# meuleman/epilogos

Hardware: NVIDIA B200
Metric: bins/sec for expected+scores (S2) (higher is better)
Workload: dtype int64+f64

## Files before the change

### epilogos_b200/csrc/common.cuh

```cuda
#pragma once
#include <cuda_runtime.h>
#include <cuda.h>
#include <stddef.h>
#include <stdint.h>
#include <stdio.h>
#include <string.h>

#include "../../include/epilogos_b200.h"

namespace epi {

void set_error(const char* fmt, ...);
int check_device();

#define EPI_CUDA(call)                                                                        \
    do {                                                                                      \
        cudaError_t e__ = (call);                                                             \
        if (e__ != cudaSuccess) {                                                             \
            epi::set_error("%s failed at %s:%d: %s", #call, __FILE__, __LINE__,               \
                           cudaGetErrorString(e__));                                          \
            return 1;                                                                         \
        }                                                                                     \
    } while (0)

#define EPI_REQUIRE(cond, ...)                                                                \
    do {                                                                                      \
        if (!(cond)) {                                                                        \
            epi::set_error(__VA_ARGS__);                                                      \
            return 2;                                                                         \
        }                                                                                     \
    } while (0)

int sm_count();
int persistent_grid(int64_t ntiles, int per_sm);

constexpr int S1_TABLE_MAX_WIDTH = 4095;

struct PrepFlags {
    int has_zero;
};

struct K5TcConsts {
    double dg[EPI_MAX_STATES];
    double scale;
    double cst;
    int has_zero;
    uint32_t m1, m8, m16;
    int fbits;
};

struct DeviceWorkspace {
    unsigned long long reduce_slots[64];
    double log2e[EPI_MAX_STATES * EPI_MAX_STATES];
    PrepFlags prep_flags;
    int s3_symmetric;
    alignas(16) uint8_t k5tc_b_image[8 * EPI_MAX_STATES * 128];
    K5TcConsts k5tc_consts;
    alignas(8) double s1_v64[EPI_MAX_STATES * (S1_TABLE_MAX_WIDTH + 1)];
    alignas(8) float s1_v32[EPI_MAX_STATES * (S1_TABLE_MAX_WIDTH + 1)];
    alignas(8) float perm_v32[2][EPI_MAX_STATES * (S1_TABLE_MAX_WIDTH + 1)];
};
static_assert(offsetof(DeviceWorkspace, k5tc_b_image) % 16 == 0, "the B operand image is a bulk-copy source");
static_assert(offsetof(DeviceWorkspace, s1_v64) % 8 == 0 && offsetof(DeviceWorkspace, s1_v32) % 8 == 0,
              "the S1 value tables need 8-byte alignment");

DeviceWorkspace* device_workspace();

typedef CUresult (*tensor_map_encode_fn)(CUtensorMap*, CUtensorMapDataType, cuuint32_t, void*, const cuuint64_t*,
                                         const cuuint64_t*, const cuuint32_t*, const cuuint32_t*,
                                         CUtensorMapInterleave, CUtensorMapSwizzle, CUtensorMapL2promotion,
                                         CUtensorMapFloatOOBfill);
tensor_map_encode_fn get_tensor_map_encode();

int s1_value_table(const float* e, int K, int width, float* v32, double* v64, cudaStream_t st);

int launch_k2_tc(const uint16_t* cnt, int64_t bins, int K, int64_t* n1, int64_t* n2, cudaStream_t st);
int scores_s2_tc(const uint16_t* cnt, int64_t bins, int K, int width, int64_t perms, const float* e, int* zero_flag,
                 float* o32, double* o64, cudaStream_t st);
bool scores_s2_tc_eligible(int width);
int scores_s2_tc_fixed_point(const float* e, int K, int64_t perms, unsigned long long* mfix_dev, int* fbits_host,
                             cudaStream_t st);

#ifdef __CUDACC__

__device__ __forceinline__ uint32_t smem_u32(const void* p) {
    return static_cast<uint32_t>(__cvta_generic_to_shared(p));
}

__device__ __forceinline__ void mbar_init(uint64_t* bar, uint32_t count) {
    asm volatile("mbarrier.init.shared::cta.b64 [%0], %1;" ::"r"(smem_u32(bar)), "r"(count));
}
__device__ __forceinline__ void mbar_fence_init() {
    asm volatile("fence.mbarrier_init.release.cluster;" ::: "memory");
}
__device__ __forceinline__ void mbar_expect_tx(uint64_t* bar, uint32_t bytes) {
    asm volatile("mbarrier.arrive.expect_tx.shared::cta.b64 _, [%0], %1;" ::"r"(smem_u32(bar)), "r"(bytes)
                 : "memory");
}
__device__ __forceinline__ void mbar_arrive(uint64_t* bar) {
    asm volatile("mbarrier.arrive.shared::cta.b64 _, [%0];" ::"r"(smem_u32(bar)) : "memory");
}
// ... 84 lines not shown
```

### epilogos_b200/csrc/count_tile.cuh

```cuda
#pragma once
#include "tc05.cuh"

namespace epi {

#ifdef __CUDACC__

constexpr int T2_OP_BYTES = 128 * 128;
constexpr int T2_DRAIN = 256;

__device__ __forceinline__ uint64_t make_mnmajor_sw128_desc(uint32_t smem_addr) {
    uint64_t d = 0;
    d |= (uint64_t)((smem_addr >> 4) & 0x3fff);
    d |= (uint64_t)((128u >> 4) & 0x3fff) << 16;
    d |= (uint64_t)((1024u >> 4) & 0x3fff) << 32;
    d |= (uint64_t)1 << 46;
    d |= (uint64_t)2 << 61;
    return d;
}
constexpr uint32_t UMMA_A_MN_MAJOR = 1u << 15, UMMA_B_MN_MAJOR = 1u << 16;

template <int KT>
__device__ __forceinline__ void store_operand_row(uint8_t* row_ptr, int r, const uint32_t (&cw)[KT / 2], int ones_word,
                                                  uint32_t ones_val) {
    constexpr int NW = ((KT / 2 + 1 + 3) / 4) * 4;
// ... 25 lines not shown
        for (int i = 0; i < NW; ++i) t[i] = w[i];
#pragma unroll
        for (int i = 0; i < KT / 2; ++i) {
            if (i < NW - 1) cw[i] = __funnelshift_r(t[i], t[i + 1], sh);
            else if (i == NW - 1) cw[i] = (sh ? (t[i] >> 16) : t[i]) & 0xffffu;
            else cw[i] = 0u;
        }
    } else {
#pragma unroll
        for (int i = 0; i < KT / 2; ++i)
            cw[i] = (2 * i < K ? (uint32_t)row[2 * i] : 0u) | ((2 * i + 1 < K ? (uint32_t)row[2 * i + 1] : 0u) << 16);
    }
}
template <int KT>
__device__ __forceinline__ void load_count_row_guarded(const uint16_t* row, int K, bool live, uint32_t (&cw)[KT / 2]) {
#pragma unroll
    for (int i = 0; i < KT / 2; ++i)
        cw[i] = (live && 2 * i < K ? (uint32_t)row[2 * i] : 0u) | ((live && 2 * i + 1 < K ? (uint32_t)row[2 * i + 1] : 0u) << 16);
}

template <int NCOL>
__device__ __forceinline__ void drain_gram(uint32_t tmem_lane_base, int warp, int lane, int K, unsigned long long* n1,
                                           unsigned long long* n2) {
    uint32_t v[NCOL];
#pragma unroll
    for (int c0 = 0; c0 < NCOL; c0 += 16) {
        uint32_t t16[16];
        tmem_ld_32x16(tmem_lane_base + (uint32_t)c0, t16);
#pragma unroll
        for (int j = 0; j < 16; ++j) v[c0 + j] = t16[j];
    }
    const int m = warp * 32 + lane;
    const int s = m >> 1;
    const bool owner = (m & 1) == 0 && s < K;
    long long diag = 0, cnt1 = 0;
#pragma unroll
    for (int q = 0; q < NCOL / 2; ++q) {
        const uint32_t p0 = __shfl_down_sync(0xffffffffu, v[2 * q], 1), p1 = __shfl_down_sync(0xffffffffu, v[2 * q + 1], 1);
        const long long val = (long long)v[2 * q] + 256ll * (long long)v[2 * q + 1] + 256ll * ((long long)p0 + 256ll * (long long)p1);
        if (q == K) cnt1 = val;
        else if (q == s) diag = val;
        else if (owner && q < K && n2 != nullptr && val != 0) atomicAdd(&n2[s * K + q], (unsigned long long)val);
    }
    if (owner) {
        diag -= cnt1;
        if (n2 != nullptr && diag != 0) atomicAdd(&n2[s * K + s], (unsigned long long)diag);
        if (n1 != nullptr && cnt1 != 0) atomicAdd(&n1[s], (unsigned long long)cnt1);
    }
}


#endif

}
```

### epilogos_b200/csrc/scores.cu

```cuda
#include "common.cuh"

namespace epi {

constexpr int K5_THREADS = 256;
constexpr int K5_WARPS = K5_THREADS / 32;
constexpr int KT_MAX = EPI_MAX_STATES;

__constant__ __align__(16) double c_log2e[KT_MAX * KT_MAX];

__global__ void k5_prepare_kernel(const float* __restrict__ e, int rows, int cols, int kt, double* __restrict__ out,
                                  PrepFlags* flags) {
    __shared__ int zero;
    if (threadIdx.x == 0) zero = 0;
    __syncthreads();
    for (int i = threadIdx.x; i < rows * kt; i += blockDim.x) {
        const int s = i / kt, q = i - s * kt;
        double v = 0.0;
        if (q < cols) {
            const double ev = (double)e[s * cols + q];
            if (ev > 0.0) v = log2(ev);
            else zero = 1;
        }
        out[i] = v;
    }
    __syncthreads();
    if (threadIdx.x == 0) flags->has_zero = zero;
}

__device__ __forceinline__ double kl_direct(double obs, double e) {
    if (e == 0.0 || obs == 0.0) return 0.0;
    return obs * log2(obs / e);
}

struct WarpCountStream {
    const uint16_t* cnt;
    uint16_t* slab[2];
    uint64_t* bar;
    long long bins, ngroups, stride;
    int K, lane, buf;
    uint32_t phase[2];

    __device__ __forceinline__ void issue(long long g, int b) const {
        if (lane == 0 && g < ngroups && bins - g * 32 >= 32) {
            mbar_expect_tx(&bar[b], 64 * K);
            bulk_load_1d(slab[b], cnt + g * 32 * K, 64 * K, &bar[b]);
        }
    }
    __device__ __forceinline__ const uint16_t* acquire(long long g, int nvalid) {
        const int b = buf;
        buf ^= 1;
        issue(g + stride, b ^ 1);
        if (nvalid == 32) {
            mbar_wait(&bar[b], phase[b]);
            phase[b] ^= 1;
// ... 76 lines not shown
        if (out32 != nullptr) warp_store_scores(myf, out32 + bin0 * K, nvalid, K, lane);
        else __syncwarp();
    }
}

__global__ void __launch_bounds__(K5_THREADS) k5_s1_direct_kernel(const uint16_t* __restrict__ cnt, long long bins, int K,
                                                                  int width, const float* __restrict__ exp1,
                                                                  float* __restrict__ out32, double* __restrict__ out64) {
    const double dw = (double)width;
    const long long n = bins * K;
    for (long long i = blockIdx.x * (long long)blockDim.x + threadIdx.x; i < n; i += (long long)gridDim.x * blockDim.x) {
        const int s = (int)(i % K);
        const double v = kl_direct((double)cnt[i] / dw, (double)__ldg(exp1 + s));
        if (out32 != nullptr) out32[i] = (float)v;
        if (out64 != nullptr) out64[i] = v;
    }
}

template <int KT>
__global__ void __launch_bounds__(K5_THREADS) k5_s2_kernel(const uint16_t* __restrict__ cnt, long long bins, int K,
                                                           int width, double perms, const float* __restrict__ exp2,
                                                           const PrepFlags* __restrict__ flags, int force_direct,
                                                           float* __restrict__ out32, double* __restrict__ out64) {
    if (force_direct == 2 && !flags->has_zero) return;
    extern __shared__ __align__(128) uint8_t smem_raw[];
    uint16_t* cslab = reinterpret_cast<uint16_t*>(smem_raw);
    float* fslab = reinterpret_cast<float*>(smem_raw + K5_WARPS * 32 * K * 4);
    uint64_t* bars = reinterpret_cast<uint64_t*>(smem_raw + K5_WARPS * 32 * K * 8);

    const int tid = threadIdx.x, warp = tid >> 5, lane = tid & 31;
    if (tid == 0) {
        for (int i = 0; i < K5_WARPS * 2; ++i) mbar_init(&bars[i], 1);
        mbar_fence_init();
    }
    __syncthreads();
    const double lp = log2(perms);
    const double inv_perms = 1.0 / perms;
    const bool direct = force_direct || flags->has_zero;
    float* myf = fslab + warp * 32 * K;

    const long long ngroups = (bins + 31) / 32;
    WarpCountStream in{cnt, {cslab + warp * 64 * K, cslab + warp * 64 * K + 32 * K}, bars + warp * 2, bins, ngroups,
                       (long long)gridDim.x * K5_WARPS, K, lane, 0, {0u, 0u}};
    in.issue((long long)blockIdx.x * K5_WARPS + warp, 0);
    for (long long g = (long long)blockIdx.x * K5_WARPS + warp; g < ngroups; g += in.stride) {
        const long long bin0 = g * 32;
        const int nvalid = (int)((bins - bin0) < 32 ? (bins - bin0) : 32);
        const uint16_t* myc = in.acquire(g, nvalid);
        if (lane < nvalid) {
            const uint16_t* row = myc + lane * K;
            float* orow = myf + lane * K;
            if (direct) {
                for (int q = 0; q < K; ++q) {
                    const long long cq = row[q];
                    double sum = 0.0;
                    if (cq != 0) {
                        for (int s = 0; s < K; ++s) {
                            const long long cs = row[s];
                            const long long prod = (s == q) ? cs * (cs - 1) : cs * cq;
                            if (prod != 0) sum += kl_direct((double)prod / perms, (double)__ldg(exp2 + s * K + q));
                        }
                    }
                    orow[q] = (float)sum;
                    if (out64 != nullptr) out64[(bin0 + lane) * K + q] = sum;
                }
            } else {
                double cd[KT], mc[KT];
                double a = 0.0, w = 0.0;
#pragma unroll
                for (int s = 0; s < KT; ++s) {
                    const int c = s < K ? row[s] : 0;
                    cd[s] = (double)c;
                    const double l = c > 0 ? log2((double)c) : 0.0;
                    a = fma(cd[s], l, a);
                    w += cd[s];
                    mc[s] = 0.0;
                }
                const double2* le2 = reinterpret_cast<const double2*>(c_log2e);
#pragma unroll
                for (int s = 0; s < KT; ++s) {
#pragma unroll
                    for (int q = 0; q < KT; q += 2) {
                        const double2 m = le2[(s * KT + q) >> 1];
                        mc[q] = fma(cd[s], m.x, mc[q]);
                        mc[q + 1] = fma(cd[s], m.y, mc[q + 1]);
                    }
                }
                const double wm1 = w - 1.0;
// ... 75 lines not shown
    }
    EPI_CUDA(cudaGetLastError());
    return 0;
}

template <int KT>
static int launch_s2(const uint16_t* cnt, int64_t bins, int K, int width, int64_t perms, const float* e,
                     const PrepFlags* flags, int direct, float* o32, double* o64, cudaStream_t st) {
    auto kern = k5_s2_kernel<KT>;
    const size_t smem = (size_t)K5_WARPS * 32 * K * 8 + K5_WARPS * 16;
    EPI_CUDA(cudaFuncSetAttribute(kern, cudaFuncAttributeMaxDynamicSharedMemorySize, (int)smem));
    const int64_t ntiles = (bins + K5_THREADS - 1) / K5_THREADS;
    kern<<<persistent_grid(ntiles, 3), K5_THREADS, smem, st>>>(cnt, bins, K, width, (double)perms, e, flags, direct, o32,
                                                                o64);
    EPI_CUDA(cudaGetLastError());
    return 0;
}

template <int KT>
static int dispatch_s2(const uint16_t* cnt, int64_t bins, int K, int width, int64_t perms, const float* e, float* o32,
                       double* o64, int mode, cudaStream_t st) {
    const PrepFlags* flags = nullptr;
    if (mode == EPI_SCORE_TABLE && scores_s2_tc_eligible(width)) {
        DeviceWorkspace* ws = device_workspace();
        EPI_REQUIRE(ws != nullptr, "could not allocate the per-device workspace");
        PrepFlags* fl = &ws->prep_flags;
        if (int rc = scores_s2_tc(cnt, bins, K, width, perms, e, &fl->has_zero, o32, o64, st)) return rc;
        return launch_s2<KT>(cnt, bins, K, width, perms, e, fl, 2, o32, o64, st);
    }
    if (int rc = prepare_tables(e, K, K, KT, st, &flags)) return rc;
    return launch_s2<KT>(cnt, bins, K, width, perms, e, flags, mode == EPI_SCORE_DIRECT, o32, o64, st);
}

}

using namespace epi;

static int check_score_args(const void* cnt, int64_t bins, int K, int width, const void* e, int mode) {
    if (check_device()) return 3;
    EPI_REQUIRE(bins >= 0 && bins < (1ll << 31), "bins=%lld out of range", (long long)bins);
    EPI_REQUIRE(K >= 1 && K <= EPI_MAX_STATES, "num_states=%d out of range [1, %d]", K, EPI_MAX_STATES);
    EPI_REQUIRE(width >= 1 && width <= 65535, "width=%d out of range [1, 65535]", width);
    EPI_REQUIRE(mode == EPI_SCORE_TABLE || mode == EPI_SCORE_DIRECT, "unknown score mode %d", mode);
    if (bins == 0) return 0;
    EPI_REQUIRE(cnt != nullptr && e != nullptr, "null pointer argument");
    EPI_REQUIRE((reinterpret_cast<uintptr_t>(cnt) & 15) == 0, "cnt_dev must be 16-byte aligned");
    return 0;
}

extern "C" int epi_scores_s1(const uint16_t* cnt_dev, int64_t bins, int32_t K, int32_t width, const float* exp1_dev,
                             float* out32_dev, double* out64_dev, int32_t mode, void* stream_) {
// ... 34 lines not shown
```

### epilogos_b200/csrc/tc_tables.cu

```cuda
#include "common.cuh"
#include "tc05.cuh"
#include "count_tile.cuh"

namespace epi {

constexpr int T2_BINS = 128;
constexpr int T2_STAGES = 4;
constexpr int T2_OPS = 2;
constexpr int T2_THREADS = 192;
constexpr int T2_TMEM_COLS = 128;

template <int KT, int KR>
__global__ void __launch_bounds__(T2_THREADS, 4)
k2_tc_kernel(const uint16_t* __restrict__ cnt, long long bins, int Krt, unsigned long long* __restrict__ n1,
             unsigned long long* __restrict__ n2) {
    const int K = KR ? KR : Krt;
    constexpr int NCOL = ((2 * KT + 1) + 15) & ~15;
    extern __shared__ uint8_t smem_raw[];
    uint8_t* smem = smem_raw + ((1024u - (smem_u32(smem_raw) & 1023u)) & 1023u);
    const int tile_bytes = T2_BINS * K * 2;
    uint8_t* ops = smem;
    uint8_t* ring = ops + T2_OPS * T2_OP_BYTES;
    uint64_t* ld_full = reinterpret_cast<uint64_t*>(ring + T2_STAGES * tile_bytes);
    uint64_t* ld_empty = ld_full + T2_STAGES;
    uint64_t* op_full = ld_empty + T2_STAGES;
    uint64_t* op_empty = op_full + T2_OPS;
    uint64_t* acc_full = op_empty + T2_OPS;
    uint64_t* acc_empty = acc_full + 1;
    uint32_t* tmem_slot = reinterpret_cast<uint32_t*>(acc_empty + 1);

    const int tid = threadIdx.x, warp = tid >> 5, lane = tid & 31;
    const long long ntiles = (bins + T2_BINS - 1) / T2_BINS;
    const long long nfull = bins / T2_BINS;

    for (int i = tid; i < T2_OPS * T2_OP_BYTES / 16; i += T2_THREADS)
        reinterpret_cast<uint4*>(ops)[i] = make_uint4(0u, 0u, 0u, 0u);
    fence_proxy_async_smem();
    if (tid == 0) {
        for (int s = 0; s < T2_STAGES; ++s) {
            mbar_init(&ld_full[s], 1);
            mbar_init(&ld_empty[s], 4);
        }
        for (int o = 0; o < T2_OPS; ++o) {
            mbar_init(&op_full[o], 4);
            mbar_init(&op_empty[o], 1);
        }
        mbar_init(acc_full, 1);
        mbar_init(acc_empty, 2);
        mbar_fence_init();
    }
    if (warp == 5) tmem_alloc(tmem_slot, T2_TMEM_COLS);
    tc_fence_before();
    __syncthreads();
    tc_fence_after();
    const uint32_t tmem_base = *tmem_slot;

    if (warp == 4) {
        if (lane == 0) {
            int i = 0;
            for (long long t = blockIdx.x; t < nfull; t += gridDim.x, ++i) {
                const int s = i % T2_STAGES;
                mbar_wait_wd(&ld_empty[s], (((uint32_t)(i / T2_STAGES)) & 1u) ^ 1u);
                mbar_expect_tx(&ld_full[s], (uint32_t)tile_bytes);
                bulk_load_1d(ring + s * tile_bytes, cnt + t * (long long)T2_BINS * K, (uint32_t)tile_bytes, &ld_full[s]);
            }
        }
    } else if (warp == 5) {
        if (lane == 0) {
            const uint32_t idesc = umma_i8_idesc(128, NCOL) | UMMA_A_MN_MAJOR | UMMA_B_MN_MAJOR;
            uint32_t acc = 0, dph = 0;
            int i = 0;
            for (long long t = blockIdx.x; t < ntiles; t += gridDim.x, ++i) {
                const int o = i % T2_OPS;
                mbar_wait_spin_wd(&op_full[o], ((uint32_t)(i / T2_OPS)) & 1u);
// ... 33 lines not shown
                                  live ? (1u << (16 * (K & 1))) : 0u);
            fence_proxy_async_smem();
            __syncwarp();
            if (lane == 0) {
                mbar_arrive(&op_full[o]);
                if (t < nfull) mbar_arrive(&ld_empty[s]);
            }

            if ((i + 1) % T2_DRAIN == 0 || t + gridDim.x >= ntiles) {
                mbar_wait_wd(acc_full, dph);
                dph ^= 1;
                tc_fence_after();
                if (warp < 2) {
                    drain_gram<NCOL>(tmem_base + ((uint32_t)(warp * 32) << 16), warp, lane, K, n1, n2);
                    tc_fence_before();
                    __syncwarp();
                    if (lane == 0) mbar_arrive(acc_empty);
                }
            }
        }
    }
    tc_fence_before();
    __syncthreads();
    if (warp == 5) tmem_dealloc(tmem_base, T2_TMEM_COLS);
}

template <int KT, int KR>
static int launch_k2_tc_impl(const uint16_t* cnt, int64_t bins, int K, int64_t* n1, int64_t* n2, cudaStream_t st) {
    const size_t smem = 1024 + (size_t)T2_OPS * T2_OP_BYTES + (size_t)T2_STAGES * T2_BINS * K * 2 +
                        (2 * T2_STAGES + 2 * T2_OPS + 2) * 8 + 16;
    auto kern = k2_tc_kernel<KT, KR>;
    EPI_CUDA(cudaFuncSetAttribute(kern, cudaFuncAttributeMaxDynamicSharedMemorySize, (int)smem));
    const int64_t ntiles = (bins + T2_BINS - 1) / T2_BINS;
    const int ctas = 4;
    kern<<<persistent_grid(ntiles, ctas), T2_THREADS, smem, st>>>(cnt, (long long)bins, K,
                                                                reinterpret_cast<unsigned long long*>(n1),
                                                                reinterpret_cast<unsigned long long*>(n2));
    EPI_CUDA(cudaGetLastError());
    return 0;
}

int launch_k2_tc(const uint16_t* cnt, int64_t bins, int K, int64_t* n1, int64_t* n2, cudaStream_t st) {
    if (K == 18) return launch_k2_tc_impl<18, 18>(cnt, bins, K, n1, n2, st);
    if (K == 15) return launch_k2_tc_impl<16, 15>(cnt, bins, K, n1, n2, st);
    if (K <= 16) return launch_k2_tc_impl<16, 0>(cnt, bins, K, n1, n2, st);
    if (K <= 18) return launch_k2_tc_impl<18, 0>(cnt, bins, K, n1, n2, st);
    return launch_k2_tc_impl<32, 0>(cnt, bins, K, n1, n2, st);
}

constexpr int T5_BINS = 128;
constexpr int T5_A_BYTES = 128 * 128;
constexpr unsigned long long T5_MAGIC = 0x4338000000000000ull;
constexpr int T5_MAX_WIDTH = 2047;

__device__ __forceinline__ unsigned long long mad_wide(uint32_t a, uint32_t b, unsigned long long c) {
    unsigned long long d;
    asm("mad.wide.u32 %0, %1, %2, %3;" : "=l"(d) : "r"(a), "r"(b), "l"(c));
    return d;
}

__device__ __forceinline__ uint32_t mad_lo(uint32_t a, uint32_t b, uint32_t c) {
    uint32_t d;
    asm("mad.lo.u32 %0, %1, %2, %3;" : "=r"(d) : "r"(a), "r"(b), "r"(c));
    return d;
}

__constant__ K5TcConsts c_k5tc;

__global__ void k5tc_prepare_kernel(const float* __restrict__ e, int K, double perms, int nrows,
                                    uint8_t* __restrict__ b_image, K5TcConsts* __restrict__ out, int* __restrict__ zero_flag,
                                    unsigned long long* __restrict__ mfix_out) {
    __shared__ unsigned long long mfix[EPI_MAX_STATES * EPI_MAX_STATES];
    __shared__ double mval[EPI_MAX_STATES * EPI_MAX_STATES];
    __shared__ unsigned long long maxbits;
    __shared__ int zero, fbits;
    if (threadIdx.x == 0) {
        maxbits = 0ull;
        zero = 0;
    }
    __syncthreads();
    for (int i = threadIdx.x; i < K * K; i += blockDim.x) {
        const double ev = (double)e[i];
        double m = 0.0;
        if (ev > 0.0) m = -log2(ev);
        else zero = 1;
        if (m < 0.0) m = 0.0;
        mval[i] = m;
        atomicMax(&maxbits, (unsigned long long)__double_as_longlong(m));
    }
    __syncthreads();
    if (threadIdx.x == 0) {
        const double mx = __longlong_as_double((long long)maxbits);
        int ib = 1;
        while (ib < 12 && (double)(1ull << ib) <= mx) ++ib;
        fbits = 56 - ib;
    }
    __syncthreads();
    const int F = fbits;
    for (int i = threadIdx.x; i < K * K; i += blockDim.x) {
        unsigned long long v = (unsigned long long)llrint(ldexp(mval[i], F));
        if (v >= (1ull << 56)) v = (1ull << 56) - 1;
        mfix[i] = v;
        if (mfix_out != nullptr) mfix_out[i] = v;
    }
    for (int i = threadIdx.x; i < nrows * 128 / 4; i += blockDim.x) reinterpret_cast<uint32_t*>(b_image)[i] = 0u;
    __syncthreads();
    for (int i = threadIdx.x; i < K * K * 14; i += blockDim.x) {
        const int dd = i % 7, h = (i / 7) & 1, st = i / 14;
        const int s = st / K, t = st - s * K;
        const uint32_t n = (uint32_t)(t * 8 + dd + h), k = (uint32_t)(2 * s + h);
        b_image[sw128_offset(n, k)] = (uint8_t)((mfix[st] >> (8 * dd)) & 255ull);
    }
    if (threadIdx.x < K) out->dg[threadIdx.x] = ldexp((double)mfix[threadIdx.x * K + threadIdx.x], -F - 3) / perms;
    if (threadIdx.x == 0) {
        const double scale = ldexp(1.0, -F) / perms;
        out->scale = scale;
        out->cst = 6755399441055744.0 * scale;
        out->has_zero = zero;
        out->m1 = 1u;
        out->m8 = 1u << 8;
        out->m16 = 1u << 16;
        out->fbits = F;
        *zero_flag = zero;
    }
}

template <int KT, int KR, int NWG, bool WANT64>
__global__ void __launch_bounds__(NWG * 128 + 64, 1)
k5_s2_tc_kernel(const uint16_t* __restrict__ cnt, long long bins, int Krt, int width, double perms,
                const uint8_t* __restrict__ b_image, float* __restrict__ out32, double* __restrict__ out64) {
    if (c_k5tc.has_zero) return;

    static_assert(KT % 2 == 0, "KT must be even");
    constexpr int NPAD = ((8 * KT + 31) / 32) * 32;
    static_assert(NPAD * NWG <= 512, "accumulator regions exceed TMEM");
    constexpr int KSTEPS = (2 * KT + 31) / 32;
    const int K = KR ? KR : Krt;

    extern __shared__ uint8_t smem_raw[];
    uint8_t* smem = smem_raw + ((1024u - (smem_u32(smem_raw) & 1023u)) & 1023u);
    const int slab_bytes = T5_BINS * K * 2;
    uint8_t* a_ops = smem;
    uint8_t* b_op = a_ops + NWG * T5_A_BYTES;
    uint8_t* slabs = b_op + NPAD * 128;
    float* stage = reinterpret_cast<float*>(slabs + NWG * 2 * slab_bytes);
    double* g1 = reinterpret_cast<double*>(stage + NWG * T5_BINS * K);
    double* f1 = g1 + ((width + 2) & ~1);
    uint64_t* ld_full = reinterpret_cast<uint64_t*>(f1 + ((width + 2) & ~1));
    uint64_t* ld_empty = ld_full + NWG * 2;
    uint64_t* a_full = ld_empty + NWG * 2;
    uint64_t* mma_done = a_full + NWG;
    uint64_t* b_full = mma_done + NWG;
    uint32_t* tmem_slot = reinterpret_cast<uint32_t*>(b_full + 1);

    const int tid = threadIdx.x, warp = tid >> 5, lane = tid & 31;
    constexpr int NT = NWG * 128 + 64;
    const long long ntiles = (bins + T5_BINS - 1) / T5_BINS;
    const long long nfull = bins / T5_BINS;

    for (int i = tid; i < NWG * T5_A_BYTES / 16; i += NT) reinterpret_cast<uint4*>(a_ops)[i] = make_uint4(0u, 0u, 0u, 0u);
    {
        const double lp = log2(perms), invp = 1.0 / perms, wm1 = (double)width - 1.0;
        for (int c = tid; c <= width; c += NT) {
            const double l = c > 0 ? log2((double)c) : 0.0;
            const double l1 = c > 1 ? log2((double)(c - 1)) : 0.0;
            const double cl = (double)c * l;
            f1[c] = cl * invp;
            g1[c] = (double)c * ((fma(l - lp, wm1, -cl) + (double)(c > 0 ? c - 1 : 0) * l1) * invp);
        }
    }
    fence_proxy_async_smem();
    if (tid == 0) {
        for (int i = 0; i < NWG * 2; ++i) {
            mbar_init(&ld_full[i], 1);
            mbar_init(&ld_empty[i], 4);
        }
        for (int g = 0; g < NWG; ++g) {
            mbar_init(&a_full[g], 4);
            mbar_init(&mma_done[g], 1);
        }
        mbar_init(b_full, 1);
        mbar_fence_init();
    }
    if (warp == 4 * NWG + 1) tmem_alloc(tmem_slot, 512);
    tc_fence_before();
    __syncthreads();
    tc_fence_after();
    const uint32_t tmem_base = *tmem_slot;

    if (warp == 4 * NWG) {
        if (lane == 0) {
            mbar_expect_tx(b_full, NPAD * 128);
            bulk_load_1d(b_op, b_image, NPAD * 128, b_full);
            int j = 0;
            for (long long t = blockIdx.x; t < nfull; t += gridDim.x, ++j) {
                const int g = j % NWG, u = j / NWG, b = u & 1;
                mbar_wait_wd(&ld_empty[g * 2 + b], (((uint32_t)(u >> 1)) & 1u) ^ 1u);
                mbar_expect_tx(&ld_full[g * 2 + b], (uint32_t)slab_bytes);
                bulk_load_1d(slabs + (g * 2 + b) * slab_bytes, cnt + t * (long long)T5_BINS * K, (uint32_t)slab_bytes,
                             &ld_full[g * 2 + b]);
            }
        }
    } else if (warp == 4 * NWG + 1) {
        if (lane == 0) {
            const uint32_t nmma = (uint32_t)((8 * K + 15) & ~15);
            const uint32_t idesc = umma_i8_idesc(128, nmma);
            mbar_wait_wd(b_full, 0);
            const uint64_t b_desc = make_kmajor_sw128_desc(smem_u32(b_op));
            int j = 0;
            for (long long t = blockIdx.x; t < ntiles; t += gridDim.x, ++j) {
                const int g = j % NWG, u = j / NWG;
                mbar_wait_spin_wd(&a_full[g], ((uint32_t)u) & 1u);
                tc_fence_after();
                const uint64_t a_desc = make_kmajor_sw128_desc(smem_u32(a_ops + g * T5_A_BYTES));
#pragma unroll
                for (int k = 0; k < KSTEPS; ++k)
                    umma_i8(tmem_base + (uint32_t)(g * NPAD), a_desc + 2 * k, b_desc + 2 * k, idesc, k ? 1u : 0u);
                umma_commit(&mma_done[g]);
            }
        }
    } else {
        const int g = warp >> 2, r = tid & 127;
        uint8_t* a_row = a_ops + g * T5_A_BYTES + r * 128;
        float* mystage = stage + g * T5_BINS * K;
        const uint32_t taddr = tmem_base + ((uint32_t)((warp & 3) * 32) << 16) + (uint32_t)(g * NPAD);
        const double scale = c_k5tc.scale * 0.125, cst = c_k5tc.cst, scale32 = c_k5tc.scale * (4294967296.0 * 0.125);
        int u = 0;
        for (long long t = blockIdx.x + (long long)g * gridDim.x; t < ntiles; t += (long long)NWG * gridDim.x, ++u) {
            const long long bin0 = t * T5_BINS;
            const int b = u & 1;
            uint32_t cw[KT / 2];
            if (t < nfull) {
                mbar_wait_wd(&ld_full[g * 2 + b], ((uint32_t)(u >> 1)) & 1u);
                load_count_row<KT, KR>(reinterpret_cast<const uint16_t*>(slabs + (g * 2 + b) * slab_bytes) + r * K, K, cw);
            } else {
                load_count_row_guarded<KT>(cnt + (bin0 + r) * K, K, bin0 + r < bins, cw);
            }
            store_operand_row<KT>(a_row, r, cw, -1, 0u);
            fence_proxy_async_smem();
            __syncwarp();
            if (lane == 0) {
                mbar_arrive(&a_full[g]);
                if (t < nfull) mbar_arrive(&ld_empty[g * 2 + b]);
            }

            uint32_t co[KT];
#pragma unroll
            for (int s = 0; s < KT; ++s) co[s] = ((cw[s >> 1] >> (16 * (s & 1))) & 0xffffu) << 3;
            double a4[4] = {0.0, 0.0, 0.0, 0.0};
// ... 2 lines not shown
            const double a_adj = (((a4[0] + a4[1]) + (a4[2] + a4[3])) - cst) * 0.125;

            if (lane == 0) bulk_wait_read0();
            __syncwarp();
            mbar_wait_wd(&mma_done[g], ((uint32_t)u) & 1u);
            tc_fence_after();
#pragma unroll
            for (int c0 = 0; c0 < 8 * KT; c0 += 32) {
                uint32_t v[32];
                double chg[4], cd[4];
#pragma unroll
                for (int i = 0; i < 4; ++i) {
                    const int tt = (c0 / 8 + i < KT) ? c0 / 8 + i : 0;
                    chg[i] = *reinterpret_cast<const double*>(reinterpret_cast<const uint8_t*>(g1) + co[tt]);
                    cd[i] = __hiloint2double(0x43300000, (int)co[tt]) - 4503599627370496.0;
                }
                tmem_ld_32x32(taddr + (uint32_t)c0, v);
                float f[4];
#pragma unroll
                for (int i = 0; i < 4; ++i) {
                    const int tt = c0 / 8 + i;
                    f[i] = 0.0f;
                    if (tt < KT && (KR == 0 || tt < KR)) {
                        const uint32_t t01 = mad_lo(v[8 * i + 1], c_k5tc.m8, v[8 * i]);
                        const uint32_t t23 = mad_lo(v[8 * i + 3], c_k5tc.m8, v[8 * i + 2]);
                        const uint32_t t45 = mad_lo(v[8 * i + 5], c_k5tc.m8, v[8 * i + 4]);
                        const uint32_t t67 = mad_lo(v[8 * i + 7], c_k5tc.m8, v[8 * i + 6]);
                        const unsigned long long lb = mad_wide(t23, c_k5tc.m16, ((unsigned long long)(T5_MAGIC >> 32) << 32) | t01);
                        const unsigned long long hb = mad_wide(t67, c_k5tc.m16, ((unsigned long long)(T5_MAGIC >> 32) << 32) | t45);
                        const double dl = __longlong_as_double((long long)lb);
                        const double dh = __longlong_as_double((long long)hb) - 6755399441055744.0;
                        const double base = fma(dh, scale32, fma(dl, scale, a_adj)) - c_k5tc.dg[tt];
                        const double val = fma(cd[i], base, chg[i]);
                        f[i] = (float)val;
                        if (WANT64 && (KR != 0 || tt < K) && bin0 + r < bins) out64[(bin0 + r) * K + tt] = val;
                    }
                }
                if constexpr (KR != 0 && KR % 2 == 0) {
                    float2* dst = reinterpret_cast<float2*>(mystage + r * KR + c0 / 8);
                    if (c0 / 8 < KR) dst[0] = make_float2(f[0], f[1]);
                    if (c0 / 8 + 2 < KR) dst[1] = make_float2(f[2], f[3]);
                } else {
#pragma unroll
                    for (int i = 0; i < 4; ++i)
                        if (c0 / 8 + i < K) mystage[r * K + c0 / 8 + i] = f[i];
                }
            }
            tc_fence_before();
            fence_proxy_async_smem();
            __syncwarp();
            if (out32 != nullptr) {
                const int wq = warp & 3;
                const long long wbin0 = bin0 + 32 * wq;
                if (t < nfull) {
                    if (lane == 0) {
                        bulk_store_1d(out32 + wbin0 * K, mystage + 32 * wq * K, (uint32_t)(32 * K * 4));
                        bulk_commit();
                    }
                } else if (wbin0 < bins) {
                    const int n = (int)((bins - wbin0) < 32 ? (bins - wbin0) : 32) * K;
                    for (int i = lane; i < n; i += 32) out32[wbin0 * K + i] = mystage[32 * wq * K + i];
                }
            }
        }
        if (lane == 0) bulk_wait0();
    }
    tc_fence_before();
    __syncthreads();
    if (warp == 4 * NWG + 1) tmem_dealloc(tmem_base, 512);
}

template <int KT, int KR, int NWG, bool WANT64>
static int launch_k5_tc2(const uint16_t* cnt, int64_t bins, int K, int width, int64_t perms, const uint8_t* b_image,
                         float* o32, double* o64, cudaStream_t st) {
    constexpr int NPAD = ((8 * KT + 31) / 32) * 32;
    auto kern = k5_s2_tc_kernel<KT, KR, NWG, WANT64>;
    const size_t smem = 1024 + (size_t)NWG * T5_A_BYTES + (size_t)NPAD * 128 + (size_t)NWG * 2 * T5_BINS * K * 2 +
                        (size_t)NWG * T5_BINS * K * 4 + (size_t)(width + 2) * 16 +
                        (size_t)(6 * NWG + 1) * 8 + 16;
    EPI_CUDA(cudaFuncSetAttribute(kern, cudaFuncAttributeMaxDynamicSharedMemorySize, (int)smem));
    const int64_t ntiles = (bins + T5_BINS - 1) / T5_BINS;
    kern<<<persistent_grid(ntiles, 1), NWG * 128 + 64, smem, st>>>(cnt, (long long)bins, K, width, (double)perms, b_image,
                                                                    o32, o64);
    EPI_CUDA(cudaGetLastError());
    return 0;
}

template <int KT, int KR, int NWG>
static int launch_k5_tc(const uint16_t* cnt, int64_t bins, int K, int width, int64_t perms, const float* e, int* zero_flag,
                        float* o32, double* o64, cudaStream_t st) {
    constexpr int NPAD = ((8 * KT + 31) / 32) * 32;
    static_assert(NPAD * 128 <= sizeof(DeviceWorkspace::k5tc_b_image), "B operand image exceeds its workspace region");
    DeviceWorkspace* ws = device_workspace();
    EPI_REQUIRE(ws != nullptr, "could not allocate the per-device workspace");
    k5tc_prepare_kernel<<<1, 256, 0, st>>>(e, K, (double)perms, NPAD, ws->k5tc_b_image, &ws->k5tc_consts, zero_flag, nullptr);
    EPI_CUDA(cudaGetLastError());
    EPI_CUDA(cudaMemcpyToSymbolAsync(c_k5tc, &ws->k5tc_consts, sizeof(K5TcConsts), 0, cudaMemcpyDeviceToDevice, st));
    if (o64 != nullptr) return launch_k5_tc2<KT, KR, NWG, true>(cnt, bins, K, width, perms, ws->k5tc_b_image, o32, o64, st);
    return launch_k5_tc2<KT, KR, NWG, false>(cnt, bins, K, width, perms, ws->k5tc_b_image, o32, o64, st);
}

int scores_s2_tc(const uint16_t* cnt, int64_t bins, int K, int width, int64_t perms, const float* e, int* zero_flag,
                 float* o32, double* o64, cudaStream_t st) {
    if (K == 18) return launch_k5_tc<18, 18, 3>(cnt, bins, K, width, perms, e, zero_flag, o32, o64, st);
    if (K == 15) return launch_k5_tc<16, 15, 4>(cnt, bins, K, width, perms, e, zero_flag, o32, o64, st);
    if (K <= 16) return launch_k5_tc<16, 0, 4>(cnt, bins, K, width, perms, e, zero_flag, o32, o64, st);
    if (K <= 18) return launch_k5_tc<18, 0, 3>(cnt, bins, K, width, perms, e, zero_flag, o32, o64, st);
    return launch_k5_tc<32, 0, 2>(cnt, bins, K, width, perms, e, zero_flag, o32, o64, st);
}

bool scores_s2_tc_eligible(int width) { return width <= T5_MAX_WIDTH; }

int scores_s2_tc_fixed_point(const float* e, int K, int64_t perms, unsigned long long* mfix_dev, int* fbits_host,
                             cudaStream_t st) {
    DeviceWorkspace* ws = device_workspace();
    EPI_REQUIRE(ws != nullptr, "could not allocate the per-device workspace");
    k5tc_prepare_kernel<<<1, 256, 0, st>>>(e, K, (double)perms, 8 * EPI_MAX_STATES, ws->k5tc_b_image, &ws->k5tc_consts,
                                           &ws->prep_flags.has_zero, mfix_dev);
    EPI_CUDA(cudaGetLastError());
    K5TcConsts host;
    EPI_CUDA(cudaMemcpyAsync(&host, &ws->k5tc_consts, sizeof(host), cudaMemcpyDeviceToHost, st));
    EPI_CUDA(cudaStreamSynchronize(st));
    if (fbits_host) *fbits_host = host.fbits;
    return 0;
}

}
```

Measured before the change: 5.182 billion.

## Fold S2 fixed-point prep and zero fallback into the tensor-core kernel

```diff
diff --git a/epilogos_b200/csrc/common.cuh b/epilogos_b200/csrc/common.cuh
--- a/epilogos_b200/csrc/common.cuh
+++ b/epilogos_b200/csrc/common.cuh
@@ -45,7 +45,6 @@
     double scale;
     double cst;
     int has_zero;
-    uint32_t m1, m8, m16;
     int fbits;
 };
 
@@ -54,13 +53,11 @@
     double log2e[EPI_MAX_STATES * EPI_MAX_STATES];
     PrepFlags prep_flags;
     int s3_symmetric;
-    alignas(16) uint8_t k5tc_b_image[8 * EPI_MAX_STATES * 128];
     K5TcConsts k5tc_consts;
     alignas(8) double s1_v64[EPI_MAX_STATES * (S1_TABLE_MAX_WIDTH + 1)];
     alignas(8) float s1_v32[EPI_MAX_STATES * (S1_TABLE_MAX_WIDTH + 1)];
     alignas(8) float perm_v32[2][EPI_MAX_STATES * (S1_TABLE_MAX_WIDTH + 1)];
 };
-static_assert(offsetof(DeviceWorkspace, k5tc_b_image) % 16 == 0, "the B operand image is a bulk-copy source");
 static_assert(offsetof(DeviceWorkspace, s1_v64) % 8 == 0 && offsetof(DeviceWorkspace, s1_v32) % 8 == 0,
               "the S1 value tables need 8-byte alignment");
 
@@ -75,8 +72,8 @@
 int s1_value_table(const float* e, int K, int width, float* v32, double* v64, cudaStream_t st);
 
 int launch_k2_tc(const uint16_t* cnt, int64_t bins, int K, int64_t* n1, int64_t* n2, cudaStream_t st);
-int scores_s2_tc(const uint16_t* cnt, int64_t bins, int K, int width, int64_t perms, const float* e, int* zero_flag,
-                 float* o32, double* o64, cudaStream_t st);
+int scores_s2_tc(const uint16_t* cnt, int64_t bins, int K, int width, int64_t perms, const float* e, float* o32,
+                 double* o64, cudaStream_t st);
 bool scores_s2_tc_eligible(int width);
 int scores_s2_tc_fixed_point(const float* e, int K, int64_t perms, unsigned long long* mfix_dev, int* fbits_host,
                              cudaStream_t st);
diff --git a/epilogos_b200/csrc/count_tile.cuh b/epilogos_b200/csrc/count_tile.cuh
--- a/epilogos_b200/csrc/count_tile.cuh
+++ b/epilogos_b200/csrc/count_tile.cuh
@@ -71,25 +71,23 @@
 template <int NCOL>
 __device__ __forceinline__ void drain_gram(uint32_t tmem_lane_base, int warp, int lane, int K, unsigned long long* n1,
                                            unsigned long long* n2) {
-    uint32_t v[NCOL];
-#pragma unroll
-    for (int c0 = 0; c0 < NCOL; c0 += 16) {
-        uint32_t t16[16];
-        tmem_ld_32x16(tmem_lane_base + (uint32_t)c0, t16);
-#pragma unroll
-        for (int j = 0; j < 16; ++j) v[c0 + j] = t16[j];
-    }
     const int m = warp * 32 + lane;
     const int s = m >> 1;
     const bool owner = (m & 1) == 0 && s < K;
     long long diag = 0, cnt1 = 0;
+#pragma unroll 1
+    for (int c0 = 0; c0 < NCOL; c0 += 16) {
+        uint32_t v[16];
+        tmem_ld_32x16(tmem_lane_base + (uint32_t)c0, v);
 #pragma unroll
-    for (int q = 0; q < NCOL / 2; ++q) {
-        const uint32_t p0 = __shfl_down_sync(0xffffffffu, v[2 * q], 1), p1 = __shfl_down_sync(0xffffffffu, v[2 * q + 1], 1);
-        const long long val = (long long)v[2 * q] + 256ll * (long long)v[2 * q + 1] + 256ll * ((long long)p0 + 256ll * (long long)p1);
-        if (q == K) cnt1 = val;
-        else if (q == s) diag = val;
-        else if (owner && q < K && n2 != nullptr && val != 0) atomicAdd(&n2[s * K + q], (unsigned long long)val);
+        for (int j = 0; j < 8; ++j) {
+            const int q = c0 / 2 + j;
+            const uint32_t p0 = __shfl_down_sync(0xffffffffu, v[2 * j], 1), p1 = __shfl_down_sync(0xffffffffu, v[2 * j + 1], 1);
+            const long long val = (long long)v[2 * j] + 256ll * (long long)v[2 * j + 1] + 256ll * ((long long)p0 + 256ll * (long long)p1);
+            if (q == K) cnt1 = val;
+            else if (q == s) diag = val;
+            else if (owner && q < K && n2 != nullptr && val != 0) atomicAdd(&n2[s * K + q], (unsigned long long)val);
+        }
     }
     if (owner) {
         diag -= cnt1;
diff --git a/epilogos_b200/csrc/s2_direct.cuh b/epilogos_b200/csrc/s2_direct.cuh
--- /dev/null
+++ b/epilogos_b200/csrc/s2_direct.cuh
@@ -0,0 +1,32 @@
+#pragma once
+#include "common.cuh"
+
+namespace epi {
+
+#ifdef __CUDACC__
+
+__device__ __forceinline__ double kl_direct(double obs, double e) {
+    if (e == 0.0 || obs == 0.0) return 0.0;
+    return obs * log2(obs / e);
+}
+
+__device__ __forceinline__ void s2_direct_row(const uint16_t* row, int K, double perms, const float* __restrict__ exp2,
+                                              float* o32, double* o64) {
+    for (int q = 0; q < K; ++q) {
+        const long long cq = row[q];
+        double sum = 0.0;
+        if (cq != 0) {
+            for (int s = 0; s < K; ++s) {
+                const long long cs = row[s];
+                const long long prod = (s == q) ? cs * (cs - 1) : cs * cq;
+                if (prod != 0) sum += kl_direct((double)prod / perms, (double)__ldg(exp2 + s * K + q));
+            }
+        }
+        if (o32 != nullptr) o32[q] = (float)sum;
+        if (o64 != nullptr) o64[q] = sum;
+    }
+}
+
+#endif
+
+}
diff --git a/epilogos_b200/csrc/scores.cu b/epilogos_b200/csrc/scores.cu
--- a/epilogos_b200/csrc/scores.cu
+++ b/epilogos_b200/csrc/scores.cu
@@ -1,4 +1,5 @@
 #include "common.cuh"
+#include "s2_direct.cuh"
 
 namespace epi {
 
@@ -25,11 +26,6 @@
     }
     __syncthreads();
     if (threadIdx.x == 0) flags->has_zero = zero;
-}
-
-__device__ __forceinline__ double kl_direct(double obs, double e) {
-    if (e == 0.0 || obs == 0.0) return 0.0;
-    return obs * log2(obs / e);
 }
 
 struct WarpCountStream {
@@ -152,7 +148,6 @@
                                                            int width, double perms, const float* __restrict__ exp2,
                                                            const PrepFlags* __restrict__ flags, int force_direct,
                                                            float* __restrict__ out32, double* __restrict__ out64) {
-    if (force_direct == 2 && !flags->has_zero) return;
     extern __shared__ __align__(128) uint8_t smem_raw[];
     uint16_t* cslab = reinterpret_cast<uint16_t*>(smem_raw);
     float* fslab = reinterpret_cast<float*>(smem_raw + K5_WARPS * 32 * K * 4);
@@ -181,19 +176,7 @@
             const uint16_t* row = myc + lane * K;
             float* orow = myf + lane * K;
             if (direct) {
-                for (int q = 0; q < K; ++q) {
-                    const long long cq = row[q];
-                    double sum = 0.0;
-                    if (cq != 0) {
-                        for (int s = 0; s < K; ++s) {
-                            const long long cs = row[s];
-                            const long long prod = (s == q) ? cs * (cs - 1) : cs * cq;
-                            if (prod != 0) sum += kl_direct((double)prod / perms, (double)__ldg(exp2 + s * K + q));
-                        }
-                    }
-                    orow[q] = (float)sum;
-                    if (out64 != nullptr) out64[(bin0 + lane) * K + q] = sum;
-                }
+                s2_direct_row(row, K, perms, exp2, orow, out64 != nullptr ? out64 + (bin0 + lane) * K : nullptr);
             } else {
                 double cd[KT], mc[KT];
                 double a = 0.0, w = 0.0;
@@ -315,11 +298,7 @@
                        double* o64, int mode, cudaStream_t st) {
     const PrepFlags* flags = nullptr;
     if (mode == EPI_SCORE_TABLE && scores_s2_tc_eligible(width)) {
-        DeviceWorkspace* ws = device_workspace();
-        EPI_REQUIRE(ws != nullptr, "could not allocate the per-device workspace");
-        PrepFlags* fl = &ws->prep_flags;
-        if (int rc = scores_s2_tc(cnt, bins, K, width, perms, e, &fl->has_zero, o32, o64, st)) return rc;
-        return launch_s2<KT>(cnt, bins, K, width, perms, e, fl, 2, o32, o64, st);
+        return scores_s2_tc(cnt, bins, K, width, perms, e, o32, o64, st);
     }
     if (int rc = prepare_tables(e, K, K, KT, st, &flags)) return rc;
     return launch_s2<KT>(cnt, bins, K, width, perms, e, flags, mode == EPI_SCORE_DIRECT, o32, o64, st);
diff --git a/epilogos_b200/csrc/tc_tables.cu b/epilogos_b200/csrc/tc_tables.cu
--- a/epilogos_b200/csrc/tc_tables.cu
+++ b/epilogos_b200/csrc/tc_tables.cu
@@ -1,21 +1,23 @@
 #include "common.cuh"
 #include "tc05.cuh"
 #include "count_tile.cuh"
+#include "s2_direct.cuh"
 
 namespace epi {
 
 constexpr int T2_BINS = 128;
-constexpr int T2_STAGES = 4;
+constexpr int T2_STAGES = 2;
 constexpr int T2_OPS = 2;
 constexpr int T2_THREADS = 192;
-constexpr int T2_TMEM_COLS = 128;
+constexpr int T2_CTAS = 5;
 
 template <int KT, int KR>
-__global__ void __launch_bounds__(T2_THREADS, 4)
+__global__ void __launch_bounds__(T2_THREADS, T2_CTAS)
 k2_tc_kernel(const uint16_t* __restrict__ cnt, long long bins, int Krt, unsigned long long* __restrict__ n1,
              unsigned long long* __restrict__ n2) {
     const int K = KR ? KR : Krt;
     constexpr int NCOL = ((2 * KT + 1) + 15) & ~15;
+    constexpr uint32_t TMEM_COLS = NCOL <= 64 ? 64 : 128;
     extern __shared__ uint8_t smem_raw[];
     uint8_t* smem = smem_raw + ((1024u - (smem_u32(smem_raw) & 1023u)) & 1023u);
     const int tile_bytes = T2_BINS * K * 2;
@@ -49,7 +51,7 @@
         mbar_init(acc_empty, 2);
         mbar_fence_init();
     }
-    if (warp == 5) tmem_alloc(tmem_slot, T2_TMEM_COLS);
+    if (warp == 5) tmem_alloc(tmem_slot, TMEM_COLS);
     tc_fence_before();
     __syncthreads();
     tc_fence_after();
@@ -129,7 +131,7 @@
     }
     tc_fence_before();
     __syncthreads();
-    if (warp == 5) tmem_dealloc(tmem_base, T2_TMEM_COLS);
+    if (warp == 5) tmem_dealloc(tmem_base, TMEM_COLS);
 }
 
 template <int KT, int KR>
@@ -139,7 +141,7 @@
     auto kern = k2_tc_kernel<KT, KR>;
     EPI_CUDA(cudaFuncSetAttribute(kern, cudaFuncAttributeMaxDynamicSharedMemorySize, (int)smem));
     const int64_t ntiles = (bins + T2_BINS - 1) / T2_BINS;
-    const int ctas = 4;
+    const int ctas = KT >= 32 ? 4 : T2_CTAS;
     kern<<<persistent_grid(ntiles, ctas), T2_THREADS, smem, st>>>(cnt, (long long)bins, K,
                                                                 reinterpret_cast<unsigned long long*>(n1),
                                                                 reinterpret_cast<unsigned long long*>(n2));
@@ -172,15 +174,13 @@
     return d;
 }
 
-__constant__ K5TcConsts c_k5tc;
-
-__global__ void k5tc_prepare_kernel(const float* __restrict__ e, int K, double perms, int nrows,
-                                    uint8_t* __restrict__ b_image, K5TcConsts* __restrict__ out, int* __restrict__ zero_flag,
-                                    unsigned long long* __restrict__ mfix_out) {
-    __shared__ unsigned long long mfix[EPI_MAX_STATES * EPI_MAX_STATES];
-    __shared__ double mval[EPI_MAX_STATES * EPI_MAX_STATES];
+__device__ __forceinline__ void k5tc_fixed_point_block(const float* __restrict__ e, int K, double perms, int nrows,
+                                                    uint8_t* b_op, unsigned long long* scratch, K5TcConsts* out,
+                                                    unsigned long long* __restrict__ mfix_out) {
     __shared__ unsigned long long maxbits;
     __shared__ int zero, fbits;
+    unsigned long long* mfix = scratch;
+    double* mval = reinterpret_cast<double*>(scratch + K * K);
     if (threadIdx.x == 0) {
         maxbits = 0ull;
         zero = 0;
@@ -210,37 +210,44 @@
         mfix[i] = v;
         if (mfix_out != nullptr) mfix_out[i] = v;
     }
-    for (int i = threadIdx.x; i < nrows * 128 / 4; i += blockDim.x) reinterpret_cast<uint32_t*>(b_image)[i] = 0u;
-    __syncthreads();
-    for (int i = threadIdx.x; i < K * K * 14; i += blockDim.x) {
-        const int dd = i % 7, h = (i / 7) & 1, st = i / 14;
-        const int s = st / K, t = st - s * K;
-        const uint32_t n = (uint32_t)(t * 8 + dd + h), k = (uint32_t)(2 * s + h);
-        b_image[sw128_offset(n, k)] = (uint8_t)((mfix[st] >> (8 * dd)) & 255ull);
-    }
+    if (b_op != nullptr)
+        for (int i = threadIdx.x; i < nrows * 128 / 16; i += blockDim.x) reinterpret_cast<uint4*>(b_op)[i] = make_uint4(0u, 0u, 0u, 0u);
+    __syncthreads();
+    if (b_op != nullptr)
+        for (int i = threadIdx.x; i < K * K * 14; i += blockDim.x) {
+            const int dd = i % 7, h = (i / 7) & 1, st = i / 14;
+            const int s = st / K, t = st - s * K;
+            const uint32_t n = (uint32_t)(t * 8 + dd + h), k = (uint32_t)(2 * s + h);
+            b_op[sw128_offset(n, k)] = (uint8_t)((mfix[st] >> (8 * dd)) & 255ull);
+        }
     if (threadIdx.x < K) out->dg[threadIdx.x] = ldexp((double)mfix[threadIdx.x * K + threadIdx.x], -F - 3) / perms;
     if (threadIdx.x == 0) {
         const double scale = ldexp(1.0, -F) / perms;
         out->scale = scale;
         out->cst = 6755399441055744.0 * scale;
         out->has_zero = zero;
-        out->m1 = 1u;
-        out->m8 = 1u << 8;
-        out->m16 = 1u << 16;
         out->fbits = F;
-        *zero_flag = zero;
-    }
+    }
+    __syncthreads();
+}
+
+__global__ void k5tc_fixed_point_kernel(const float* __restrict__ e, int K, double perms, K5TcConsts* __restrict__ out,
+                                        unsigned long long* __restrict__ mfix_out) {
+    __shared__ unsigned long long scratch[2 * EPI_MAX_STATES * EPI_MAX_STATES];
+    __shared__ K5TcConsts consts;
+    k5tc_fixed_point_block(e, K, perms, 0, nullptr, scratch, &consts, mfix_out);
+    if (threadIdx.x == 0) *out = consts;
 }
 
 template <int KT, int KR, int NWG, bool WANT64>
 __global__ void __launch_bounds__(NWG * 128 + 64, 1)
 k5_s2_tc_kernel(const uint16_t* __restrict__ cnt, long long bins, int Krt, int width, double perms,
-                const uint8_t* __restrict__ b_image, float* __restrict__ out32, double* __restrict__ out64) {
-    if (c_k5tc.has_zero) return;
-
+                const float* __restrict__ e, uint32_t m8, uint32_t m16, float* __restrict__ out32,
+                double* __restrict__ out64) {
     static_assert(KT % 2 == 0, "KT must be even");
     constexpr int NPAD = ((8 * KT + 31) / 32) * 32;
     static_assert(NPAD * NWG <= 512, "accumulator regions exceed TMEM");
+    static_assert(16 * KT * KT <= NWG * T5_A_BYTES, "prologue scratch exceeds the A operand buffers");
     constexpr int KSTEPS = (2 * KT + 31) / 32;
     const int K = KR ? KR : Krt;
 
@@ -253,20 +260,22 @@
     float* stage = reinterpret_cast<float*>(slabs + NWG * 2 * slab_bytes);
     double* g1 = reinterpret_cast<double*>(stage + NWG * T5_BINS * K);
     double* f1 = g1 + ((width + 2) & ~1);
-    uint64_t* ld_full = reinterpret_cast<uint64_t*>(f1 + ((width + 2) & ~1));
+    K5TcConsts* kc = reinterpret_cast<K5TcConsts*>(f1 + ((width + 2) & ~1));
+    uint64_t* ld_full = reinterpret_cast<uint64_t*>(kc + 1);
     uint64_t* ld_empty = ld_full + NWG * 2;
     uint64_t* a_full = ld_empty + NWG * 2;
     uint64_t* mma_done = a_full + NWG;
-    uint64_t* b_full = mma_done + NWG;
-    uint32_t* tmem_slot = reinterpret_cast<uint32_t*>(b_full + 1);
+    uint32_t* tmem_slot = reinterpret_cast<uint32_t*>(mma_done + NWG);
 
     const int tid = threadIdx.x, warp = tid >> 5, lane = tid & 31;
     constexpr int NT = NWG * 128 + 64;
     const long long ntiles = (bins + T5_BINS - 1) / T5_BINS;
     const long long nfull = bins / T5_BINS;
 
+    k5tc_fixed_point_block(e, K, perms, NPAD, b_op, reinterpret_cast<unsigned long long*>(a_ops), kc, nullptr);
+    const bool has_zero = kc->has_zero != 0;
     for (int i = tid; i < NWG * T5_A_BYTES / 16; i += NT) reinterpret_cast<uint4*>(a_ops)[i] = make_uint4(0u, 0u, 0u, 0u);
-    {
+    if (!has_zero) {
         const double lp = log2(perms), invp = 1.0 / perms, wm1 = (double)width - 1.0;
         for (int c = tid; c <= width; c += NT) {
             const double l = c > 0 ? log2((double)c) : 0.0;
@@ -286,7 +295,6 @@
             mbar_init(&a_full[g], 4);
             mbar_init(&mma_done[g], 1);
         }
-        mbar_init(b_full, 1);
         mbar_fence_init();
     }
     if (warp == 4 * NWG + 1) tmem_alloc(tmem_slot, 512);
@@ -295,10 +303,12 @@
     tc_fence_after();
     const uint32_t tmem_base = *tmem_slot;
 
-    if (warp == 4 * NWG) {
+    if (has_zero) {
+        for (long long b = (long long)blockIdx.x * NT + tid; b < bins; b += (long long)gridDim.x * NT)
+            s2_direct_row(cnt + b * K, K, perms, e, out32 != nullptr ? out32 + b * K : nullptr,
+                          out64 != nullptr ? out64 + b * K : nullptr);
+    } else if (warp == 4 * NWG) {
         if (lane == 0) {
-            mbar_expect_tx(b_full, NPAD * 128);
-            bulk_load_1d(b_op, b_image, NPAD * 128, b_full);
             int j = 0;
             for (long long t = blockIdx.x; t < nfull; t += gridDim.x, ++j) {
                 const int g = j % NWG, u = j / NWG, b = u & 1;
@@ -312,7 +322,6 @@
         if (lane == 0) {
             const uint32_t nmma = (uint32_t)((8 * K + 15) & ~15);
             const uint32_t idesc = umma_i8_idesc(128, nmma);
-            mbar_wait_wd(b_full, 0);
             const uint64_t b_desc = make_kmajor_sw128_desc(smem_u32(b_op));
             int j = 0;
             for (long long t = blockIdx.x; t < ntiles; t += gridDim.x, ++j) {
@@ -331,7 +340,8 @@
         uint8_t* a_row = a_ops + g * T5_A_BYTES + r * 128;
         float* mystage = stage + g * T5_BINS * K;
         const uint32_t taddr = tmem_base + ((uint32_t)((warp & 3) * 32) << 16) + (uint32_t)(g * NPAD);
-        const double scale = c_k5tc.scale * 0.125, cst = c_k5tc.cst, scale32 = c_k5tc.scale * (4294967296.0 * 0.125);
+        const double scale = kc->scale * 0.125, cst = kc->cst, scale32 = kc->scale * (4294967296.0 * 0.125);
+        const double* dg = kc->dg;
         int u = 0;
         for (long long t = blockIdx.x + (long long)g * gridDim.x; t < ntiles; t += (long long)NWG * gridDim.x, ++u) {
             const long long bin0 = t * T5_BINS;
@@ -380,15 +390,15 @@
                     const int tt = c0 / 8 + i;
                     f[i] = 0.0f;
                     if (tt < KT && (KR == 0 || tt < KR)) {
-                        const uint32_t t01 = mad_lo(v[8 * i + 1], c_k5tc.m8, v[8 * i]);
-                        const uint32_t t23 = mad_lo(v[8 * i + 3], c_k5tc.m8, v[8 * i + 2]);
-                        const uint32_t t45 = mad_lo(v[8 * i + 5], c_k5tc.m8, v[8 * i + 4]);
-                        const uint32_t t67 = mad_lo(v[8 * i + 7], c_k5tc.m8, v[8 * i + 6]);
-                        const unsigned long long lb = mad_wide(t23, c_k5tc.m16, ((unsigned long long)(T5_MAGIC >> 32) << 32) | t01);
-                        const unsigned long long hb = mad_wide(t67, c_k5tc.m16, ((unsigned long long)(T5_MAGIC >> 32) << 32) | t45);
+                        const uint32_t t01 = mad_lo(v[8 * i + 1], m8, v[8 * i]);
+                        const uint32_t t23 = mad_lo(v[8 * i + 3], m8, v[8 * i + 2]);
+                        const uint32_t t45 = mad_lo(v[8 * i + 5], m8, v[8 * i + 4]);
+                        const uint32_t t67 = mad_lo(v[8 * i + 7], m8, v[8 * i + 6]);
+                        const unsigned long long lb = mad_wide(t23, m16, ((unsigned long long)(T5_MAGIC >> 32) << 32) | t01);
+                        const unsigned long long hb = mad_wide(t67, m16, ((unsigned long long)(T5_MAGIC >> 32) << 32) | t45);
                         const double dl = __longlong_as_double((long long)lb);
                         const double dh = __longlong_as_double((long long)hb) - 6755399441055744.0;
-                        const double base = fma(dh, scale32, fma(dl, scale, a_adj)) - c_k5tc.dg[tt];
+                        const double base = fma(dh, scale32, fma(dl, scale, a_adj)) - dg[tt];
                         const double val = fma(cd[i], base, chg[i]);
                         f[i] = (float)val;
                         if (WANT64 && (KR != 0 || tt < K) && bin0 + r < bins) out64[(bin0 + r) * K + tt] = val;
@@ -429,42 +439,35 @@
 }
 
 template <int KT, int KR, int NWG, bool WANT64>
-static int launch_k5_tc2(const uint16_t* cnt, int64_t bins, int K, int width, int64_t perms, const uint8_t* b_image,
-                         float* o32, double* o64, cudaStream_t st) {
+static int launch_k5_tc2(const uint16_t* cnt, int64_t bins, int K, int width, int64_t perms, const float* e, float* o32,
+                         double* o64, cudaStream_t st) {
     constexpr int NPAD = ((8 * KT + 31) / 32) * 32;
     auto kern = k5_s2_tc_kernel<KT, KR, NWG, WANT64>;
     const size_t smem = 1024 + (size_t)NWG * T5_A_BYTES + (size_t)NPAD * 128 + (size_t)NWG * 2 * T5_BINS * K * 2 +
-                        (size_t)NWG * T5_BINS * K * 4 + (size_t)(width + 2) * 16 +
-                        (size_t)(6 * NWG + 1) * 8 + 16;
+                        (size_t)NWG * T5_BINS * K * 4 + (size_t)(width + 2) * 16 + sizeof(K5TcConsts) +
+                        (size_t)(6 * NWG) * 8 + 16;
     EPI_CUDA(cudaFuncSetAttribute(kern, cudaFuncAttributeMaxDynamicSharedMemorySize, (int)smem));
     const int64_t ntiles = (bins + T5_BINS - 1) / T5_BINS;
-    kern<<<persistent_grid(ntiles, 1), NWG * 128 + 64, smem, st>>>(cnt, (long long)bins, K, width, (double)perms, b_image,
-                                                                    o32, o64);
+    kern<<<persistent_grid(ntiles, 1), NWG * 128 + 64, smem, st>>>(cnt, (long long)bins, K, width, (double)perms, e,
+                                                                    1u << 8, 1u << 16, o32, o64);
     EPI_CUDA(cudaGetLastError());
     return 0;
 }
 
 template <int KT, int KR, int NWG>
-static int launch_k5_tc(const uint16_t* cnt, int64_t bins, int K, int width, int64_t perms, const float* e, int* zero_flag,
-                        float* o32, double* o64, cudaStream_t st) {
-    constexpr int NPAD = ((8 * KT + 31) / 32) * 32;
-    static_assert(NPAD * 128 <= sizeof(DeviceWorkspace::k5tc_b_image), "B operand image exceeds its workspace region");
-    DeviceWorkspace* ws = device_workspace();
-    EPI_REQUIRE(ws != nullptr, "could not allocate the per-device workspace");
-    k5tc_prepare_kernel<<<1, 256, 0, st>>>(e, K, (double)perms, NPAD, ws->k5tc_b_image, &ws->k5tc_consts, zero_flag, nullptr);
-    EPI_CUDA(cudaGetLastError());
-    EPI_CUDA(cudaMemcpyToSymbolAsync(c_k5tc, &ws->k5tc_consts, sizeof(K5TcConsts), 0, cudaMemcpyDeviceToDevice, st));
-    if (o64 != nullptr) return launch_k5_tc2<KT, KR, NWG, true>(cnt, bins, K, width, perms, ws->k5tc_b_image, o32, o64, st);
-    return launch_k5_tc2<KT, KR, NWG, false>(cnt, bins, K, width, perms, ws->k5tc_b_image, o32, o64, st);
-}
-
-int scores_s2_tc(const uint16_t* cnt, int64_t bins, int K, int width, int64_t perms, const float* e, int* zero_flag,
-                 float* o32, double* o64, cudaStream_t st) {
-    if (K == 18) return launch_k5_tc<18, 18, 3>(cnt, bins, K, width, perms, e, zero_flag, o32, o64, st);
-    if (K == 15) return launch_k5_tc<16, 15, 4>(cnt, bins, K, width, perms, e, zero_flag, o32, o64, st);
-    if (K <= 16) return launch_k5_tc<16, 0, 4>(cnt, bins, K, width, perms, e, zero_flag, o32, o64, st);
-    if (K <= 18) return launch_k5_tc<18, 0, 3>(cnt, bins, K, width, perms, e, zero_flag, o32, o64, st);
-    return launch_k5_tc<32, 0, 2>(cnt, bins, K, width, perms, e, zero_flag, o32, o64, st);
+static int launch_k5_tc(const uint16_t* cnt, int64_t bins, int K, int width, int64_t perms, const float* e, float* o32,
+                        double* o64, cudaStream_t st) {
+    if (o64 != nullptr) return launch_k5_tc2<KT, KR, NWG, true>(cnt, bins, K, width, perms, e, o32, o64, st);
+    return launch_k5_tc2<KT, KR, NWG, false>(cnt, bins, K, width, perms, e, o32, o64, st);
+}
+
+int scores_s2_tc(const uint16_t* cnt, int64_t bins, int K, int width, int64_t perms, const float* e, float* o32,
+                 double* o64, cudaStream_t st) {
+    if (K == 18) return launch_k5_tc<18, 18, 3>(cnt, bins, K, width, perms, e, o32, o64, st);
+    if (K == 15) return launch_k5_tc<16, 15, 4>(cnt, bins, K, width, perms, e, o32, o64, st);
+    if (K <= 16) return launch_k5_tc<16, 0, 4>(cnt, bins, K, width, perms, e, o32, o64, st);
+    if (K <= 18) return launch_k5_tc<18, 0, 3>(cnt, bins, K, width, perms, e, o32, o64, st);
+    return launch_k5_tc<32, 0, 2>(cnt, bins, K, width, perms, e, o32, o64, st);
 }
 
 bool scores_s2_tc_eligible(int width) { return width <= T5_MAX_WIDTH; }
@@ -473,8 +476,7 @@
                              cudaStream_t st) {
     DeviceWorkspace* ws = device_workspace();
     EPI_REQUIRE(ws != nullptr, "could not allocate the per-device workspace");
-    k5tc_prepare_kernel<<<1, 256, 0, st>>>(e, K, (double)perms, 8 * EPI_MAX_STATES, ws->k5tc_b_image, &ws->k5tc_consts,
-                                           &ws->prep_flags.has_zero, mfix_dev);
+    k5tc_fixed_point_kernel<<<1, 256, 0, st>>>(e, K, (double)perms, &ws->k5tc_consts, mfix_dev);
     EPI_CUDA(cudaGetLastError());
     K5TcConsts host;
     EPI_CUDA(cudaMemcpyAsync(&host, &ws->k5tc_consts, sizeof(host), cudaMemcpyDeviceToHost, st));
```

Result: no change. 5.155 billion, median of 6 (-0.5%).
